# Kmatsuo57/cell-image-analysis

Measured on NVIDIA B200. Metric: cells scored/sec (crop+resize+CAE+SVM), higher is better.
Workload: dtype f16 tensor cores (CAE, PCA, SVM cross term: fp16 hi+lo operands, fp32 accumulate) / f64 norms and sums

## Files before the change

### cell-image-analysis_b200/csrc/cae_tc.cu

```cuda
#include "common.cuh"
#include "tc_ptx.cuh"

#include <cuda.h>
#include <cuda_fp16.h>

#include <cmath>

namespace {

constexpr int TCT = 256;
enum { EPI_POOL = 0, EPI_PLAIN = 2, EPI_FINAL = 3, EPI_PHASE = 4 };

using namespace tcptx;

#ifdef CIA_LANE0_ISSUE
#define ISSUE_WARP(cond) (lane == 0 && (cond))
#define ISSUE_BEGIN {
#define ISSUE_END }
#else
#define ISSUE_WARP(cond) (cond)
#define ISSUE_BEGIN if (elect_one()) {
#define ISSUE_END } __syncwarp();
#endif
#ifdef CIA_SPIN_WAIT
#define MBAR_WAIT mbar_wait
#else
#define MBAR_WAIT mbar_wait_sleep
#endif
#ifdef CIA_SLEEP_WAIT_ALL
#define mbar_wait mbar_wait_sleep
#endif
#ifdef CIA_UNIFORM_ISSUE_ALL
#define ISSUE1_WARP(cond) (cond)
#define ISSUE1_BEGIN if (elect_one()) {
#define ISSUE1_END } __syncwarp();
#else
#define ISSUE1_WARP(cond) (lane == 0 && (cond))
#define ISSUE1_BEGIN {
#define ISSUE1_END }
#endif

__device__ __forceinline__ float pooled_act(float folded_max, float inv_scale, float invd, float b, float s, float t) {
    const float m = __uint_as_float(__float_as_uint(folded_max) ^ (__float_as_uint(s) & 0x80000000u));
    return __fadd_rn(__fmul_rn(fmaxf(fmaf(m, inv_scale, fmaf(m, invd, b)), 0.f), s), t);
}

__device__ __forceinline__ void split_store8(const float (&o)[8], __half* hi_dst, __half* lo_dst, bool& range_ok) {
    __align__(16) __half hh[8];
    __align__(16) __half ll[8];
#pragma unroll
    for (int k = 0; k < 8; ++k) {
        hh[k] = __float2half_rn(o[k]);
        ll[k] = __float2half_rn(o[k] - __half2float(hh[k]));
        range_ok = range_ok && fabsf(o[k]) < 65520.f;
    }
    *reinterpret_cast<uint4*>(hi_dst) = *reinterpret_cast<const uint4*>(hh);
    if (lo_dst) *reinterpret_cast<uint4*>(lo_dst) = *reinterpret_cast<const uint4*>(ll);
}

template <int CIN, int COUT, int R, int EPI, int NPASS>
struct Cfg {
    static constexpr bool POOL = EPI == EPI_POOL;
    static constexpr int NCH = CIN / 8;
    static constexpr int FILL_ROWS = POOL ? R + 2 : 18;
    static constexpr int UNIT_COLS = (R >= 32 && CIN >= 64) ? 16 : R;
    static constexpr int COL_BLOCKS = R / UNIT_COLS;
    static constexpr int ROW_UNITS = POOL ? 9 : UNIT_COLS + 2;
    static constexpr int ROW_B = ROW_UNITS * 16;
    static constexpr int PLANE_B = FILL_ROWS * ROW_B;
    static constexpr int CHUNK_B = (POOL ? 2 : 1) * PLANE_B;
    static constexpr int REGION_B = NCH * CHUNK_B;
    static constexpr int SBO_A = POOL ? 2 * ROW_B : ROW_B;
    static constexpr int TILES = POOL ? 4 : (UNIT_COLS >= 8 ? UNIT_COLS / 8 : 1);
    static constexpr int UNITS_PER_CELL = POOL ? (R >= 32 ? 2 : 1) : (R >= 32 ? 2 : 1) * COL_BLOCKS;
    static constexpr int TBUF_COLS = TILES * COUT;
    static constexpr int TMEM_COLS = pow2_cols((NPASS == 1 ? 2 : 1) * TBUF_COLS);
    static constexpr int W_B = 9 * NCH * COUT * 16;
    static constexpr int PARTS = NPASS > 1 ? 2 : 1;
    static constexpr int SMEM_B = PARTS * (REGION_B + W_B);
    static constexpr bool DED_ISSUER = NPASS == 1 && !POOL && EPI != EPI_FINAL && SMEM_B > 100 * 1024;
    static constexpr int THREADS = TCT + (DED_ISSUER ? 32 : 0);
};

template <class C, int R, int NPASS, int NT, int BATCH, bool UPSIN = false>
__device__ __forceinline__ void stage_block(const __half* __restrict__ in_hi, const __half* __restrict__ in_lo,
                                            unsigned char* a0, unsigned char* a1, int cell, int sub, int tid) {
    constexpr int COLS = C::POOL ? 18 : C::ROW_UNITS;
    constexpr int N_UNITS16 = C::NCH * C::FILL_ROWS * COLS;
    constexpr int ITERS = (N_UNITS16 + NT - 1) / NT;
#pragma unroll 1
    for (int i0 = 0; i0 < ITERS; i0 += BATCH) {
        uint4 vh[BATCH], vl[BATCH];
        uint32_t dst[BATCH];
#pragma unroll
        for (int j = 0; j < BATCH; ++j) {
            const int idx = tid + (i0 + j) * NT;
            vh[j] = make_uint4(0, 0, 0, 0); vl[j] = make_uint4(0, 0, 0, 0);
            dst[j] = 0xFFFFFFFFu;
            if (i0 + j < ITERS && idx < N_UNITS16) {
                const int c = idx / (C::FILL_ROWS * COLS);
                const int rem = idx - c * (C::FILL_ROWS * COLS);
                const int ry = rem / COLS, rc = rem - ry * COLS;
                int y, x;
                if (C::POOL) {
                    y = ry - 1; x = 16 * sub - 1 + rc;
                    dst[j] = (uint32_t)(((c * 2 + (rc & 1)) * C::FILL_ROWS + ry) * 9 + (rc >> 1)) * 16u;
                } else {
                    y = 16 * (sub / C::COL_BLOCKS) + ry - 1;
                    x = C::UNIT_COLS * (sub % C::COL_BLOCKS) + rc - 1;
                    dst[j] = (uint32_t)((c * C::FILL_ROWS + ry) * C::ROW_UNITS + rc) * 16u;
                }
                if (y >= 0 && y < R && x >= 0 && x < R) {
                    constexpr int RS = UPSIN ? R / 2 : R;
                    const int ys = UPSIN ? (y >> 1) : y, xs = UPSIN ? (x >> 1) : x;
                    const size_t src = ((((size_t)cell * C::NCH + c) * RS + ys) * RS + xs);
                    vh[j] = __ldg(reinterpret_cast<const uint4*>(in_hi) + src);
                    if (NPASS > 1) vl[j] = __ldg(reinterpret_cast<const uint4*>(in_lo) + src);
                }
            }
        }
#pragma unroll
        for (int j = 0; j < BATCH; ++j) {
            if (dst[j] != 0xFFFFFFFFu) {
                *reinterpret_cast<uint4*>(a0 + dst[j]) = vh[j];
                if (NPASS > 1) *reinterpret_cast<uint4*>(a1 + dst[j]) = vl[j];
            }
        }
    }
}

template <int CIN, int COUT, int R, int EPI, int NPASS, bool UPSIN>
__global__ void __launch_bounds__(Cfg<CIN, COUT, R, EPI, NPASS>::THREADS, (Cfg<CIN, COUT, R, EPI, NPASS>::SMEM_B > 100 * 1024) ? 1 : 2)
conv_tc_kernel(const __half* __restrict__ in_hi, const __half* __restrict__ in_lo,
               const uint4* __restrict__ w_hi, const uint4* __restrict__ w_lo, float inv_scale,
               const float* __restrict__ bias, const float* __restrict__ bn_s,
               const float* __restrict__ bn_t, __half* __restrict__ out_hi, __half* __restrict__ out_lo,
               float* __restrict__ feat, const float* __restrict__ crops, float* __restrict__ mse,
               float* __restrict__ mae, int n_cells, const int32_t* __restrict__ n_dev, int cell0,
               int chunk_cells,
               int32_t* __restrict__ status) {
    bool range_ok = true;
    using C = Cfg<CIN, COUT, R, EPI, NPASS>;
    extern __shared__ __align__(1024) unsigned char smem[];
    __shared__ __align__(8) uint64_t bar[2];
    __shared__ uint32_t tmem_base_s;
    __shared__ float red_s[2][2][TCT / 32];

    const int tid = threadIdx.x, warp = tid >> 5, lane = tid & 31;
    unsigned char* a_part[2] = {smem, smem + C::REGION_B};
    unsigned char* w_part[2] = {smem + C::PARTS * C::REGION_B, smem + C::PARTS * C::REGION_B + C::W_B};

    int n = dev_count(n_cells, n_dev) - cell0;
    if (n > chunk_cells) n = chunk_cells;
    if (n <= 0) return;
    const int n_units = n * C::UNITS_PER_CELL;

    if (warp == 0) tmem_alloc(&tmem_base_s, C::TMEM_COLS);
    constexpr int NISS = C::DED_ISSUER ? 1 : C::TILES;
    if (tid == 32) { mbar_init(&bar[0], NISS); mbar_init(&bar[1], NISS); fence_barrier_init(); }
    for (int i = tid; i < C::W_B / 16; i += TCT) {
        reinterpret_cast<uint4*>(w_part[0])[i] = __ldg(w_hi + i);
        if (NPASS > 1) reinterpret_cast<uint4*>(w_part[1])[i] = __ldg(w_lo + i);
    }
    tc_fence_before();
    __syncthreads();
    tc_fence_after();
    const uint32_t tmem_base = tmem_base_s;
    constexpr uint32_t IDESC = make_idesc(128, COUT);

    constexpr int S_COLS = C::POOL ? 18 : C::ROW_UNITS;
    constexpr int S_N = C::NCH * C::FILL_ROWS * S_COLS;
    constexpr int S_IT = (S_N + TCT - 1) / TCT;
    constexpr bool PIPE = NPASS == 1;
    uint32_t s_dst[S_IT], s_crc[S_IT];
    uint4 s_val[S_IT];
    if (PIPE) {
#pragma unroll
        for (int j = 0; j < S_IT; ++j) {
            const int idx = tid + j * TCT;
            s_dst[j] = 0xFFFFFFFFu; s_crc[j] = 0;
            if (idx < S_N && tid < TCT) {
                const int c = idx / (C::FILL_ROWS * S_COLS);
                const int rem = idx - c * (C::FILL_ROWS * S_COLS);
                const int ry = rem / S_COLS, rc = rem - ry * S_COLS;
                s_crc[j] = (uint32_t)((c << 16) | (ry << 8) | rc);
                s_dst[j] = C::POOL ? (uint32_t)(((c * 2 + (rc & 1)) * C::FILL_ROWS + ry) * 9 + (rc >> 1)) * 16u
                                   : (uint32_t)((c * C::FILL_ROWS + ry) * C::ROW_UNITS + rc) * 16u;
            }
        }
    }
    auto prefetch = [&](int unit) {
        const int cell = cell0 + unit / C::UNITS_PER_CELL;
        const int sub = unit % C::UNITS_PER_CELL;
        const int y0 = C::POOL ? -1 : 16 * (sub / C::COL_BLOCKS) - 1;
        const int x0 = C::POOL ? 16 * sub - 1 : C::UNIT_COLS * (sub % C::COL_BLOCKS) - 1;
        constexpr int RS = UPSIN ? R / 2 : R;
        const uint4* base = reinterpret_cast<const uint4*>(in_hi) + (size_t)cell * C::NCH * RS * RS;
#pragma unroll
        for (int j = 0; j < S_IT; ++j) {
            const int c = (int)(s_crc[j] >> 16), y = y0 + (int)((s_crc[j] >> 8) & 255u), x = x0 + (int)(s_crc[j] & 255u);
            s_val[j] = make_uint4(0, 0, 0, 0);
            if (s_dst[j] != 0xFFFFFFFFu && y >= 0 && y < R && x >= 0 && x < R) {
                const int ys = UPSIN ? (y >> 1) : y, xs = UPSIN ? (x >> 1) : x;
                s_val[j] = __ldg(base + ((size_t)c * RS + ys) * RS + xs);
            }
        }
    };
    auto park = [&]() {
#pragma unroll
// ... 1302 lines not shown
}

namespace l7 {
constexpr int EPI_WARPS = 16;
constexpr int NT = (EPI_WARPS + 1) * 32;
constexpr int A_B = 1024 * 32 * 2;
constexpr int W_B = 4 * 32 * 16;
constexpr int PL_B = 16 * 1024 * 4;
constexpr int SMEM_B = 2 * A_B + W_B + PL_B;
constexpr int STAGE_COLS = 8 * 32;
}

__global__ void __launch_bounds__(l7::NT, 1)
final_tapsum_kernel(const __half* __restrict__ a6, const uint4* __restrict__ w_img, float inv_scale,
                    const float* __restrict__ bias, const float* __restrict__ crops,
                    float* __restrict__ mse, float* __restrict__ mae, int n_cells,
                    const int32_t* __restrict__ n_dev, int cell0, int chunk_cells) {
    using namespace l7;
    extern __shared__ __align__(1024) unsigned char smem[];
    __shared__ __align__(8) uint64_t a_full[2], d_full[2], d_empty[2];
    __shared__ uint32_t tmem_base_s;
    __shared__ float red_s[2][2][EPI_WARPS];
    unsigned char* const w_s = smem + 2 * A_B;
    float* const planes = reinterpret_cast<float*>(smem + 2 * A_B + W_B);

    const int tid = threadIdx.x, warp = tid >> 5, lane = tid & 31;
    int n = dev_count(n_cells, n_dev) - cell0;
    if (n > chunk_cells) n = chunk_cells;
    if (n <= 0) return;
    const int stride = (int)gridDim.x;

    if (warp == 0) tmem_alloc(&tmem_base_s, 2 * STAGE_COLS);
    if (tid == 32) {
        for (int i = 0; i < 2; ++i) { mbar_init(&a_full[i], 1); mbar_init(&d_full[i], 1); mbar_init(&d_empty[i], EPI_WARPS); }
        fence_barrier_init();
    }
    for (int i = tid; i < W_B / 16; i += NT) reinterpret_cast<uint4*>(w_s)[i] = __ldg(w_img + i);
    fence_async_smem();
    tc_fence_before();
    __syncthreads();
    tc_fence_after();
    const uint32_t tmem_base = tmem_base_s;

    if (warp == EPI_WARPS) {
        if (ISSUE1_WARP(true)) {
            constexpr uint32_t IDESC = make_idesc(128, 32);
            const uint64_t bd0 = make_smem_desc(smem_u32(w_s), 32 * 16, 128);
            const __half* src0 = a6 + (size_t)cell0 * (A_B / 2);
            ISSUE1_BEGIN
            for (int k = 0; k < 2; ++k) {
                const int unit = (int)blockIdx.x + k * stride;
                if (unit < n) {
                    mbar_expect_tx(&a_full[k], A_B);
                    bulk_load(smem_u32(smem) + k * A_B, src0 + (size_t)unit * (A_B / 2), A_B, &a_full[k]);
                }
            }
            ISSUE1_END
            uint32_t it = 0;
            for (int unit = blockIdx.x; unit < n; unit += stride, ++it) {
                const uint32_t st = it & 1, ph = (it >> 1) & 1;
                mbar_wait(&a_full[st], ph);
                mbar_wait(&d_empty[st], ph ^ 1);
                tc_fence_after();
                ISSUE1_BEGIN
                const uint64_t ad0 = make_smem_desc(smem_u32(smem) + st * A_B, 1024 * 16, 128);
#pragma unroll
                for (int t = 0; t < 8; ++t)
#pragma unroll
                    for (int ks = 0; ks < 2; ++ks)
                        umma_f16(tmem_base + st * STAGE_COLS + (uint32_t)(t * 32),
                                 ad0 + (uint64_t)((t * 128 * 16 + 2 * ks * 1024 * 16) >> 4),
                                 bd0 + (uint64_t)((2 * ks * 32 * 16) >> 4), IDESC, ks);
                umma_commit(&d_full[st]);
                ISSUE1_END
                mbar_wait(&d_full[st], ph);
                if (unit + 2 * stride < n) {
                    ISSUE1_BEGIN
                    mbar_expect_tx(&a_full[st], A_B);
                    bulk_load(smem_u32(smem) + st * A_B, src0 + (size_t)(unit + 2 * stride) * (A_B / 2), A_B, &a_full[st]);
                    ISSUE1_END
                }
            }
        }
    } else {
        const int q = warp & 3, g = warp >> 2;
        const float b = __ldg(bias);
        uint32_t it = 0;
        for (int unit = blockIdx.x; unit < n; unit += stride, ++it) {
            const uint32_t st = it & 1, ph = (it >> 1) & 1;
            const int cell = cell0 + unit;
            mbar_wait(&d_full[st], ph);
            tc_fence_after();
#pragma unroll
            for (int tt = 0; tt < 2; ++tt) {
                const int t = g + 4 * tt;
                const int p = 128 * t + 32 * q + lane;
                const uint32_t taddr = tmem_base + ((uint32_t)(32 * q) << 16) + st * STAGE_COLS + (uint32_t)(t * 32);
                uint32_t v[4][8];
#pragma unroll
                for (int k = 0; k < 4; ++k) TMEM_LD8(taddr + 8 * k, v[k]);
#pragma unroll
                for (int k = 0; k < 4; ++k) TMEM_WAIT8(v[k]);
#pragma unroll
                for (int c = 0; c < 16; ++c)
                    planes[c * 1024 + p] = __uint_as_float(v[c >> 3][c & 7]) + __uint_as_float(v[2 + (c >> 3)][c & 7]);
            }
            tc_fence_before();
            __syncwarp();
            if (lane == 0) mbar_arrive(&d_empty[st]);
            asm volatile("bar.sync 1, %0;" ::"n"(EPI_WARPS * 32) : "memory");
            float se = 0.f, ae = 0.f;
            const float* xr = crops + (size_t)cell * 4096;
#pragma unroll
            for (int tt = 0; tt < 2; ++tt) {
                const int p = 128 * (g + 4 * tt) + 32 * q + lane;
                const int Y = p >> 5, X = p & 31;
#pragma unroll
                for (int py = 0; py < 2; ++py) {
                    const float2 xv = __ldg(reinterpret_cast<const float2*>(xr + (2 * Y + py) * 64 + 2 * X));
#pragma unroll
                    for (int px = 0; px < 2; ++px) {
                        float sum = 0.f;
#pragma unroll
                        for (int ty = 0; ty < 2; ++ty)
#pragma unroll
                            for (int tx = 0; tx < 2; ++tx) {
                                const int yy = Y + py - 1 + ty, xx = X + px - 1 + tx;
                                if ((unsigned)yy < 32u && (unsigned)xx < 32u)
                                    sum += planes[(4 * (2 * py + px) + 2 * ty + tx) * 1024 + yy * 32 + xx];
                            }
                        const float a = fmaf(sum, inv_scale, b);
                        const float rec = __fdividef(1.f, 1.f + __expf(-a));
                        const float d = (px ? xv.y : xv.x) - rec;
                        se = fmaf(d, d, se);
                        ae += fabsf(d);
                    }
                }
            }
            se = warp_sum(se); ae = warp_sum(ae);
            if (lane == 0) { red_s[it & 1][0][warp] = se; red_s[it & 1][1][warp] = ae; }
            asm volatile("bar.sync 1, %0;" ::"n"(EPI_WARPS * 32) : "memory");
            if (tid == 0) {
                float s = 0.f, a = 0.f;
#pragma unroll
                for (int w = 0; w < EPI_WARPS; ++w) { s += red_s[it & 1][0][w]; a += red_s[it & 1][1][w]; }
                mse[cell] = s * (1.f / 4096.f);
                mae[cell] = a * (1.f / 4096.f);
            }
        }
    }
    tc_fence_before();
    __syncthreads();
    if (warp == 0) tmem_dealloc(tmem_base, 2 * l7::STAGE_COLS);
}

template <int CIN, int COUT, int R, int EPI, int NPASS, bool UPSIN = false>
int launch_tc(cia_ctx* h, const CaeWeights& w, int layer, const __half* in_hi, const __half* in_lo,
              __half* out_hi, __half* out_lo, float* feat, const float* crops, float* mse, float* mae,
              int n, const int32_t* n_dev, int cell0, int chunk, cudaStream_t s) {
    using C = Cfg<CIN, COUT, R, EPI, NPASS>;
    auto kern = conv_tc_kernel<CIN, COUT, R, EPI, NPASS, UPSIN>;
    if (first_use(h, (const void*)kern))
        CIA_CUDA(cudaFuncSetAttribute(kern, cudaFuncAttributeMaxDynamicSharedMemorySize, C::SMEM_B));
    int grid = chunk * C::UNITS_PER_CELL;
    const int cap = h->num_sms * (C::SMEM_B > 100 * 1024 ? 1 : 2);
    if (grid > cap) grid = cap;
    kern<<<grid, C::THREADS, C::SMEM_B, s>>>(in_hi, in_lo, (const uint4*)w.tc_w[layer][0], (const uint4*)w.tc_w[layer][1],
                                      w.tc_inv_scale[layer], w.bias[layer], w.bn_scale[layer], w.bn_shift[layer],
                                      out_hi, out_lo, feat, crops, mse, mae, n, n_dev, cell0, chunk, h->status_dev);
    CIA_LAUNCH_CHECK();
    return CIA_OK;
}

#ifdef CIA_ACC_TIMING
static void acc_timing_dump(const char* name, int cin, int cout, int r, int g, cudaStream_t s) {
    if (!getenv("CIA_ACC_DUMP")) return;
    unsigned long long d[16];
    cudaStreamSynchronize(s);
    cudaMemcpyFromSymbol(d, g_acc_dbg, sizeof(d));
    const double u = d[5] ? (double)d[5] : 1.0;
    fprintf(stderr, "%s<%d,%d,%d,G%d> cells %llu per-cell cycles: stage %.0f wait_full %.0f ld %.0f ld+add %.0f "
                    "final %.0f | mma: wait_ready %.0f wait_empty %.0f issue %.0f\n", name, cin, cout, r, g, d[5],
            d[0] / u, d[1] / u, d[2] / u, d[3] / u, d[4] / u, d[8] / u, d[9] / u, d[10] / u);
    memset(d, 0, sizeof(d));
    cudaMemcpyToSymbol(g_acc_dbg, d, sizeof(d));
}
#else
static inline void acc_timing_dump(const char*, int, int, int, int, cudaStream_t) {}
#endif

static float acc_debias(const cia_ctx* h, int layer) { return h->cae_debias[layer == 1 ? 1 : 2] * 5.9604645e-8f; }

template <int CIN, int COUT, int R, int G = 1>
int launch_tc_acc(cia_ctx* h, const CaeWeights& w, int layer, const __half* in_hi, const __half* in_lo,
                  __half* out_hi, __half* out_lo, float* feat, int n, const int32_t* n_dev, int cell0,
                  int chunk, cudaStream_t s) {
    using C = AccCfg<CIN, COUT, R>;
    auto kern = conv_tc_acc_kernel<CIN, COUT, R, G>;
    if (first_use(h, (const void*)kern))
        CIA_CUDA(cudaFuncSetAttribute(kern, cudaFuncAttributeMaxDynamicSharedMemorySize, C::SMEM_B));
    int grid = chunk;
    if (grid > h->num_sms) grid = h->num_sms;
    kern<<<grid, ACC_THREADS, C::SMEM_B, s>>>(in_hi, in_lo, (const uint4*)w.tc_w[layer][0],
                                              (const uint4*)w.tc_w[layer][1], w.tc_inv_scale[layer],
                                              w.tc_inv_scale[layer] * acc_debias(h, layer), w.bias[layer],
                                              w.bn_scale[layer], w.bn_shift[layer], out_hi, out_lo, feat, n, n_dev,
                                              cell0, chunk, h->status_dev);
    CIA_LAUNCH_CHECK();
    acc_timing_dump("acc", CIN, COUT, R, G, s);
    return CIA_OK;
}

typedef CUresult (*TensorMapEncodeFn)(CUtensorMap*, CUtensorMapDataType, cuuint32_t, void*, const cuuint64_t*,
                                      const cuuint64_t*, const cuuint32_t*, const cuuint32_t*, CUtensorMapInterleave,
                                      CUtensorMapSwizzle, CUtensorMapL2promotion, CUtensorMapFloatOOBfill);

static int encode_act_map(cia_ctx* h, CUtensorMap* tm, const __half* base, int nch, int r, int cells, int box_x,
                          int box_y) {
    static TensorMapEncodeFn encode = [] {
        void* fn = nullptr;
        cudaDriverEntryPointQueryResult q;
        if (cudaGetDriverEntryPoint("cuTensorMapEncodeTiled", &fn, cudaEnableDefault, &q) != cudaSuccess) fn = nullptr;
        return (TensorMapEncodeFn)fn;
    }();
    if (!encode) { h->err = "cuTensorMapEncodeTiled is not available from this driver"; return CIA_E_UNSUPPORTED; }
    const cuuint64_t dims[5] = {8, (cuuint64_t)r, (cuuint64_t)r, (cuuint64_t)nch, (cuuint64_t)cells};
    const cuuint64_t strides[4] = {16, (cuuint64_t)16 * r, (cuuint64_t)16 * r * r, (cuuint64_t)16 * r * r * nch};
    const cuuint32_t box[5] = {8, (cuuint32_t)box_x, (cuuint32_t)box_y, (cuuint32_t)nch, 1};
    const cuuint32_t estr[5] = {1, 2, 1, 1, 1};
    const CUresult rc = encode(tm, CU_TENSOR_MAP_DATA_TYPE_FLOAT16, 5, (void*)base, dims, strides, box, estr,
                               CU_TENSOR_MAP_INTERLEAVE_NONE, CU_TENSOR_MAP_SWIZZLE_NONE,
                               CU_TENSOR_MAP_L2_PROMOTION_L2_128B, CU_TENSOR_MAP_FLOAT_OOB_FILL_NONE);
    if (rc != CUDA_SUCCESS) { h->err = "cuTensorMapEncodeTiled failed"; return CIA_E_CUDA; }
    return CIA_OK;
}

template <int CIN, int COUT, int R, int G>
int launch_tc_acc2(cia_ctx* h, const CaeWeights& w, int layer, const __half* in_hi, const __half* in_lo,
                   int buf_cells, __half* out_hi, __half* out_lo, float* feat, int n, const int32_t* n_dev,
                   int cell0, int chunk, cudaStream_t s) {
    using C = Acc2Cfg<CIN, COUT, R>;
    static_assert(C::SMEM_B + 1280 <= 227 * 1024, "double-buffered blocks do not fit in shared memory");
    auto kern = conv_tc_acc2_kernel<CIN, COUT, R, G>;
    if (first_use(h, (const void*)kern))
        CIA_CUDA(cudaFuncSetAttribute(kern, cudaFuncAttributeMaxDynamicSharedMemorySize, C::SMEM_B));
    CUtensorMap tm_hi, tm_lo;
    int rc;
    if ((rc = encode_act_map(h, &tm_hi, in_hi, C::NCH, C::R, buf_cells, C::BOX_X, C::FILL_ROWS))) return rc;
    if ((rc = encode_act_map(h, &tm_lo, in_lo, C::NCH, C::R, buf_cells, C::BOX_X, C::FILL_ROWS))) return rc;
    int grid = chunk;
    if (grid > h->num_sms) grid = h->num_sms;
    kern<<<grid, ACC_THREADS, C::SMEM_B, s>>>(tm_hi, tm_lo, (const uint4*)w.tc_w[layer][0],
                                              (const uint4*)w.tc_w[layer][1], w.tc_inv_scale[layer],
                                              w.tc_inv_scale[layer] * acc_debias(h, layer), w.bias[layer],
                                              w.bn_scale[layer], w.bn_shift[layer], out_hi, out_lo, feat, n, n_dev,
                                              cell0, chunk, h->status_dev);
    CIA_LAUNCH_CHECK();
    acc_timing_dump("acc2", CIN, COUT, R, G, s);
    return CIA_OK;
}

template <int G, int VAR = 0>
int launch_l2_stack(cia_ctx* h, const CaeWeights& w, const __half* in_hi, const __half* in_lo, int buf_cells,
                    __half* out_hi, __half* out_lo, float* feat, int n, const int32_t* n_dev, int cell0, int chunk,
                    cudaStream_t s) {
    using C = Acc2Cfg<32, 64, 32>;
    auto kern = conv_tc_l2_stack_kernel<G, VAR>;
    if (first_use(h, (const void*)kern))
        CIA_CUDA(cudaFuncSetAttribute(kern, cudaFuncAttributeMaxDynamicSharedMemorySize, C::SMEM_B));
    CUtensorMap tm_hi, tm_lo;
    int rc;
    if ((rc = encode_act_map(h, &tm_hi, in_hi, C::NCH, C::R, buf_cells, C::BOX_X, C::FILL_ROWS))) return rc;
    if ((rc = encode_act_map(h, &tm_lo, in_lo, C::NCH, C::R, buf_cells, C::BOX_X, C::FILL_ROWS))) return rc;
    int grid = chunk;
    if (grid > h->num_sms) grid = h->num_sms;
    kern<<<grid, ACC_THREADS, C::SMEM_B, s>>>(tm_hi, tm_lo, (const uint4*)w.tc_w[1][0], (const uint4*)w.tc_w[1][1],
                                              w.tc_inv_scale[1], w.tc_inv_scale[1] * acc_debias(h, 1), w.bias[1],
                                              w.bn_scale[1], w.bn_shift[1], out_hi, out_lo, feat, n, n_dev, cell0, chunk, h->status_dev);
    CIA_LAUNCH_CHECK();
    return CIA_OK;
}

static void pack_image(const std::vector<float>& w , int taps, int cin, int N,
                       int n_real, int sw, std::vector<__half>& hi, std::vector<__half>& lo,
                       const float* colsign = nullptr) {
    const int nch = cin / 8;
    hi.assign((size_t)taps * nch * N * 8, __float2half_rn(0.f));
    lo = hi;
    const float sc = std::ldexp(1.f, sw);
    for (int tap = 0; tap < taps; ++tap)
        for (int c = 0; c < cin; ++c)
            for (int nn = 0; nn < n_real; ++nn) {
                const float v = w[((size_t)tap * cin + c) * n_real + nn] * sc * (colsign ? colsign[nn] : 1.f);
                const __half hv = __float2half_rn(v);
                const size_t idx = (((size_t)tap * nch + c / 8) * N + nn) * 8 + (c % 8);
                hi[idx] = hv;
                lo[idx] = __float2half_rn(v - __half2float(hv));
            }
}

static int scale_exp(const std::vector<float>& w) {
    float m = 0.f;
    for (float v : w) m = std::fmax(m, std::fabs(v));
    if (!(m > 0.f)) return 0;
    int e;
    std::frexp(m, &e);
// ... 61 lines not shown
                                    kt[(size_t)c * 16 + 4 * (2 * py + px) + 2 * ty + tx] += k[((size_t)(dy * 3 + dx) * cin + c)];
                            }
                std::vector<__half> img((size_t)(cin / 8) * 32 * 8, __float2half_rn(0.f));
                const float sc = std::ldexp(1.f, sw);
                for (int c = 0; c < cin; ++c)
                    for (int col = 0; col < 16; ++col) {
                        const float v = kt[(size_t)c * 16 + col] * sc;
                        const __half hv = __float2half_rn(v);
                        img[((size_t)(c / 8) * 32 + col) * 8 + (c % 8)] = hv;
                        img[((size_t)(c / 8) * 32 + 16 + col) * 8 + (c % 8)] = __float2half_rn(v - __half2float(hv));
                    }
                cudaFree(w.tc_w7); w.tc_w7 = nullptr;
                CIA_CUDA(cudaMalloc(&w.tc_w7, img.size() * sizeof(__half)));
                CIA_CUDA(cudaMemcpy(w.tc_w7, img.data(), img.size() * sizeof(__half), cudaMemcpyHostToDevice));
            }
        } else if (L == 5) {
            const int N = 4 * cout;
            std::vector<float> kp((size_t)9 * cin * N, 0.f);
            for (int py = 0; py < 2; ++py)
                for (int px = 0; px < 2; ++px)
                    for (int dy = 0; dy < 3; ++dy)
                        for (int dx = 0; dx < 3; ++dx) {
                            const int oy = (int)std::floor((py + dy - 1) / 2.0), ox = (int)std::floor((px + dx - 1) / 2.0);
                            const int tl = (oy + 1) * 3 + (ox + 1);
                            for (int c = 0; c < cin; ++c)
                                for (int co = 0; co < cout; ++co)
                                    kp[((size_t)tl * cin + c) * N + (py * 2 + px) * cout + co] +=
                                        k[((size_t)(dy * 3 + dx) * cin + c) * cout + co];
                        }
            sw = scale_exp(kp);
            pack_image(kp, 9, cin, N, N, sw, hi, lo);
        } else {
            sw = scale_exp(k);
            pack_image(k, 9, cin, cout, cout, sw, hi, lo, L < 3 ? colsign.data() : nullptr);
        }
        w.tc_inv_scale[L] = std::ldexp(1.f, -sw);
        for (int j = 0; j < 2; ++j) {
            cudaFree(w.tc_w[L][j]); w.tc_w[L][j] = nullptr;
            const std::vector<__half>& src = j == 0 ? hi : lo;
            CIA_CUDA(cudaMalloc(&w.tc_w[L][j], src.size() * sizeof(__half)));
            CIA_CUDA(cudaMemcpy(w.tc_w[L][j], src.data(), src.size() * sizeof(__half), cudaMemcpyHostToDevice));
        }
    }
    w.tc_ready = true;
    return CIA_OK;
}

int k_cae_forward_tc(cia_ctx* h, const float* crops, int n, const int32_t* n_dev, float* mse,
                     float* mae, float* features, int mode, cudaStream_t s) {
    if (n <= 0) return CIA_OK;
    const CaeWeights& ae = h->cae[0];
    if (!ae.loaded || ae.n_conv != 7 || !ae.tc_ready) { h->err = "cia_cae_forward: autoencoder not loaded"; return CIA_E_STATE; }
    const bool sep = h->cae[1].loaded;
    const bool tc_feat = mode == 1 && !sep;
    const bool l3_exact = mode == 3 && !sep;
    const int CH_MAX = h->cae_pass_cells;
    const int CH = n < CH_MAX ? (n + 147) / 148 * 148 : CH_MAX;
    const size_t a1 = 4 * 32 * 32 * 8, a2 = 8 * 16 * 16 * 8, a3 = 4 * 8 * 8 * 8, a4u = 4 * 8 * 8 * 8,
                 a5u = 8 * 16 * 16 * 8, a6 = 4 * 32 * 32 * 8;
    const size_t per_cell = 2 * a1 + 2 * a2 + a3 + a4u + a5u + a6;
    int rc = ws_reserve(h, h->ws_misc, (size_t)CH * per_cell * sizeof(__half));
    if (rc) return rc;
    float* A2f = nullptr;
    if (l3_exact) {
        if ((rc = ws_reserve(h, h->ws_act, (size_t)CH * 16 * 16 * 64 * sizeof(float)))) return rc;
        A2f = (float*)h->ws_act.p;
    }
    __half* A1h = (__half*)h->ws_misc.p;
    __half* A1l = A1h + CH * a1;
    __half* A2h = A1l + CH * a1;
    __half* A2l = A2h + CH * a2;
    __half* A3h = A2l + CH * a2;
    __half* A4u = A3h + CH * a3;
    __half* A5u = A4u + CH * a4u;
    __half* A6 = A5u + CH * a5u;
    CIA_CUDA(cudaMemsetAsync(mse, 0, (size_t)n * sizeof(float), s));
    CIA_CUDA(cudaMemsetAsync(mae, 0, (size_t)n * sizeof(float), s));
    const bool side_encoder = features && !tc_feat && !l3_exact;
    if (side_encoder) {
        CIA_CUDA(cudaEventRecord(h->ev_fork, s));
        CIA_CUDA(cudaStreamWaitEvent(h->side, h->ev_fork, 0));
        rc = k_encoder_fp32(h, sep ? h->cae[1] : h->cae[0], crops, n, n_dev, features, h->side);
        if (rc) return rc;
        CIA_CUDA(cudaEventRecord(h->ev_join, h->side));
    }
    for (int c0 = 0; c0 < n; c0 += CH) {
        const int chunk = (n - c0) < CH ? (n - c0) : CH;
        __half* a1h = A1h - (size_t)c0 * a1; __half* a1l = A1l - (size_t)c0 * a1;
        __half* a2h = A2h - (size_t)c0 * a2; __half* a2l = A2l - (size_t)c0 * a2;
        __half* a3h = A3h - (size_t)c0 * a3; __half* a4 = A4u - (size_t)c0 * a4u;
        __half* a5 = A5u - (size_t)c0 * a5u; __half* a6p = A6 - (size_t)c0 * a6;
        float* feat = tc_feat ? features : nullptr;
        int grid1 = chunk * 4;
        if (grid1 > h->num_sms * 8) grid1 = h->num_sms * 8;
        const int pass = c0 / CH;
        if (h->layer_ev && pass < CIA_LAYER_PASSES) h->layer_passes = pass + 1;
#define CIA_LMARK(i) do { if (h->layer_ev && pass < CIA_LAYER_PASSES) CIA_CUDA(cudaEventRecord(h->layer_ev[pass * CIA_LAYER_MARKS + (i)], s)); } while (0)
        CIA_LMARK(0);
        if (tc_feat || l3_exact) {
            static const int l1_tc = [] { const char* e = getenv("CIA_L1_KERNEL"); return e ? atoi(e) : 1; }();
            const float l1_debias = h->cae_debias[0] * 5.9604645e-8f;
            if (l1_tc) {
                if (first_use(h, (const void*)conv1_tc_split_kernel))
                    CIA_CUDA(cudaFuncSetAttribute(conv1_tc_split_kernel, cudaFuncAttributeMaxDynamicSharedMemorySize, l1tc::SMEM_B));
                int gridt = chunk * 8;
                if (gridt > h->num_sms * 2) gridt = h->num_sms * 2;
                conv1_tc_split_kernel<<<gridt, l1tc::NT, l1tc::SMEM_B, s>>>(crops, (const uint4*)ae.tc_w[0][0], ae.tc_inv_scale[0],
                                                                            l1_debias, ae.bias[0], ae.bn_scale[0], ae.bn_shift[0],
                                                                            a1h, a1l, n, n_dev, c0, chunk, h->status_dev);
            } else {
                conv1_fp32_planar_kernel<<<grid1, 256, 0, s>>>(crops, ae.kernel[0], ae.bias[0], ae.bn_scale[0],
                                                               ae.bn_shift[0], a1h, a1l, n, n_dev, c0, chunk, h->status_dev);
            }
            CIA_LAUNCH_CHECK();
            CIA_LMARK(1);
            float* a2f = l3_exact ? A2f - (size_t)c0 * (16 * 16 * 64) : nullptr;
            static const int l2_g = [] { const char* e = getenv("CIA_L2_TAPS_PER_FLUSH"); return e ? atoi(e) : 3; }();
            static const int l2_stack = [] { const char* e = getenv("CIA_L2_STACK"); return e ? atoi(e) : 0; }();
            if (l2_stack == 2 && l2_g == 3) rc = launch_l2_stack<3, 1>(h, ae, A1h, A1l, CH, a2h, a2l, a2f, n, n_dev, c0, chunk, s);
            else if (l2_stack == 3 && l2_g == 3) rc = launch_l2_stack<3, 2>(h, ae, A1h, A1l, CH, a2h, a2l, a2f, n, n_dev, c0, chunk, s);
            else if (l2_stack && l2_g == 3) rc = launch_l2_stack<3>(h, ae, A1h, A1l, CH, a2h, a2l, a2f, n, n_dev, c0, chunk, s);
            else if (l2_g == 0) rc = launch_tc_acc<32, 64, 32, 1>(h, ae, 1, a1h, a1l, a2h, a2l, a2f, n, n_dev, c0, chunk, s);
            else if (l2_g == 1) rc = launch_tc_acc2<32, 64, 32, 1>(h, ae, 1, A1h, A1l, CH, a2h, a2l, a2f, n, n_dev, c0, chunk, s);
            else if (l2_g == 9) rc = launch_tc_acc2<32, 64, 32, 9>(h, ae, 1, A1h, A1l, CH, a2h, a2l, a2f, n, n_dev, c0, chunk, s);
            else if (l2_g == 2) rc = launch_tc_acc2<32, 64, 32, 2>(h, ae, 1, A1h, A1l, CH, a2h, a2l, a2f, n, n_dev, c0, chunk, s);
            else rc = launch_tc_acc2<32, 64, 32, 3>(h, ae, 1, A1h, A1l, CH, a2h, a2l, a2f, n, n_dev, c0, chunk, s);
            if (rc) return rc;
            CIA_LMARK(2);
            if (l3_exact) {
                if ((rc = launch_tc<64, 32, 16, EPI_POOL, 1>(h, ae, 2, a2h, nullptr, a3h, nullptr, nullptr, nullptr, nullptr, nullptr, n, n_dev, c0, chunk, s))) return rc;
                if (features && (rc = k_conv3_fp32(h, ae, a2f, n, n_dev, features, c0, chunk, s))) return rc;
            } else {
                static const int l3_tma = [] { const char* e = getenv("CIA_L3_KERNEL"); return e ? atoi(e) : 0; }();
                static const int l3_g = [] { const char* e = getenv("CIA_L3_TAPS_PER_FLUSH"); return e ? atoi(e) : 1; }();
                if (l3_tma) rc = launch_tc_acc2<64, 32, 16, 1>(h, ae, 2, A2h, A2l, CH, a3h, nullptr, feat, n, n_dev, c0, chunk, s);
                else if (l3_g == 3) rc = launch_tc_acc<64, 32, 16, 3>(h, ae, 2, a2h, a2l, a3h, nullptr, feat, n, n_dev, c0, chunk, s);
                else rc = launch_tc_acc<64, 32, 16, 1>(h, ae, 2, a2h, a2l, a3h, nullptr, feat, n, n_dev, c0, chunk, s);
                if (rc) return rc;
            }
        } else {
            conv1_fp32_planar_kernel<<<grid1, 256, 0, s>>>(crops, ae.kernel[0], ae.bias[0], ae.bn_scale[0],
                                                           ae.bn_shift[0], a1h, nullptr, n, n_dev, c0, chunk, h->status_dev);
            CIA_LAUNCH_CHECK();
            CIA_LMARK(1);
            if ((rc = launch_tc<32, 64, 32, EPI_POOL, 1>(h, ae, 1, a1h, nullptr, a2h, nullptr, nullptr, nullptr, nullptr, nullptr, n, n_dev, c0, chunk, s))) return rc;
            CIA_LMARK(2);
            if ((rc = launch_tc<64, 32, 16, EPI_POOL, 1>(h, ae, 2, a2h, nullptr, a3h, nullptr, nullptr, nullptr, nullptr, nullptr, n, n_dev, c0, chunk, s))) return rc;
        }
        CIA_LMARK(3);
        if ((rc = launch_tc<32, 32, 8, EPI_PLAIN, 1>(h, ae, 3, a3h, nullptr, a4, nullptr, nullptr, nullptr, nullptr, nullptr, n, n_dev, c0, chunk, s))) return rc;
        CIA_LMARK(4);
        if ((rc = launch_tc<32, 64, 16, EPI_PLAIN, 1, true>(h, ae, 4, a4, nullptr, a5, nullptr, nullptr, nullptr, nullptr, nullptr, n, n_dev, c0, chunk, s))) return rc;
        CIA_LMARK(5);
        if ((rc = launch_tc<64, 128, 16, EPI_PHASE, 1>(h, ae, 5, a5, nullptr, a6p, nullptr, nullptr, nullptr, nullptr, nullptr, n, n_dev, c0, chunk, s))) return rc;
        CIA_LMARK(6);
        static const int l7_tapsum = [] { const char* e = getenv("CIA_L7_KERNEL"); return e ? atoi(e) : 1; }();
        if (l7_tapsum) {
            if (first_use(h, (const void*)final_tapsum_kernel))
                CIA_CUDA(cudaFuncSetAttribute(final_tapsum_kernel, cudaFuncAttributeMaxDynamicSharedMemorySize, l7::SMEM_B));
            int g7 = chunk < h->num_sms ? chunk : h->num_sms;
            final_tapsum_kernel<<<g7, l7::NT, l7::SMEM_B, s>>>(a6p, (const uint4*)ae.tc_w7, ae.tc_inv_scale[6], ae.bias[6],
                                                              crops, mse, mae, n, n_dev, c0, chunk);
            CIA_LAUNCH_CHECK();
        } else if ((rc = launch_tc<32, 16, 32, EPI_FINAL, 1>(h, ae, 6, a6p, nullptr, nullptr, nullptr, nullptr, crops, mse, mae, n, n_dev, c0, chunk, s))) return rc;
        CIA_LMARK(7);
#undef CIA_LMARK
    }
    if (side_encoder) CIA_CUDA(cudaStreamWaitEvent(s, h->ev_join, 0));
    return CIA_OK;
}
```

### cell-image-analysis_b200/csrc/tc_ptx.cuh

```cuda
#pragma once
#include <cuda_runtime.h>
#include <stdint.h>

namespace tcptx {

__device__ __forceinline__ uint32_t smem_u32(const void* p) { return (uint32_t)__cvta_generic_to_shared(p); }

__device__ __forceinline__ void mbar_init(uint64_t* bar, uint32_t count) {
    asm volatile("mbarrier.init.shared::cta.b64 [%0], %1;" ::"r"(smem_u32(bar)), "r"(count) : "memory");
}
__device__ __forceinline__ void mbar_wait(uint64_t* bar, uint32_t parity) {
    const uint32_t a = smem_u32(bar);
    uint32_t done;
    do {
        asm volatile(
            "{\n\t.reg .pred p;\n\t"
            "mbarrier.try_wait.parity.shared::cta.b64 p, [%1], %2;\n\t"
            "selp.u32 %0, 1, 0, p;\n\t}"
            : "=r"(done) : "r"(a), "r"(parity) : "memory");
    } while (!done);
}
__device__ __forceinline__ void mbar_wait_sleep(uint64_t* bar, uint32_t parity) {
    const uint32_t a = smem_u32(bar);
    asm volatile(
        "{\n\t.reg .pred p;\n\t"
        "WAIT_%=:\n\t"
        "mbarrier.try_wait.parity.shared::cta.b64 p, [%0], %1, %2;\n\t"
        "@p bra DONE_%=;\n\t"
        "bra WAIT_%=;\n\t"
        "DONE_%=:\n\t}"
        ::"r"(a), "r"(parity), "r"(0x989680u) : "memory");
}
__device__ __forceinline__ bool elect_one() {
    uint32_t pred;
    asm volatile("{\n\t.reg .pred p;\n\telect.sync _|p, 0xffffffff;\n\tselp.u32 %0, 1, 0, p;\n\t}" : "=r"(pred));
    return pred != 0;
}
__device__ __forceinline__ void fence_barrier_init() { asm volatile("fence.mbarrier_init.release.cluster;" ::: "memory"); }
__device__ __forceinline__ void fence_async_smem() { asm volatile("fence.proxy.async.shared::cta;" ::: "memory"); }
__device__ __forceinline__ void tc_fence_before() { asm volatile("tcgen05.fence::before_thread_sync;" ::: "memory"); }
__device__ __forceinline__ void tc_fence_after() { asm volatile("tcgen05.fence::after_thread_sync;" ::: "memory"); }

__device__ __forceinline__ void tmem_alloc(uint32_t* dst_smem, uint32_t ncols) {
    asm volatile("tcgen05.alloc.cta_group::1.sync.aligned.shared::cta.b32 [%0], %1;" ::"r"(smem_u32(dst_smem)), "r"(ncols) : "memory");
    asm volatile("tcgen05.relinquish_alloc_permit.cta_group::1.sync.aligned;" ::: "memory");
}
__device__ __forceinline__ void tmem_dealloc(uint32_t taddr, uint32_t ncols) {
    asm volatile("tcgen05.dealloc.cta_group::1.sync.aligned.b32 %0, %1;" ::"r"(taddr), "r"(ncols) : "memory");
}
__device__ __forceinline__ void umma_f16(uint32_t d_tmem, uint64_t adesc, uint64_t bdesc, uint32_t idesc,
                                         uint32_t accumulate) {
    asm volatile(
        "{\n\t.reg .pred p;\n\tsetp.ne.b32 p, %4, 0;\n\t"
        "tcgen05.mma.cta_group::1.kind::f16 [%0], %1, %2, %3, p;\n\t}"
        ::"r"(d_tmem), "l"(adesc), "l"(bdesc), "r"(idesc), "r"(accumulate) : "memory");
}
__device__ __forceinline__ void umma_commit(uint64_t* bar) {
    asm volatile("tcgen05.commit.cta_group::1.mbarrier::arrive::one.shared::cluster.b64 [%0];" ::"r"(smem_u32(bar)) : "memory");
}
#define TMEM_LD8(taddr, v)                                                                          \
    asm volatile("tcgen05.ld.sync.aligned.32x32b.x8.b32 {%0,%1,%2,%3,%4,%5,%6,%7}, [%8];"            \
                 : "=r"(v[0]), "=r"(v[1]), "=r"(v[2]), "=r"(v[3]), "=r"(v[4]), "=r"(v[5]), "=r"(v[6]), \
                   "=r"(v[7]) : "r"(taddr))
#define TMEM_WAIT8(v)                                                                               \
    asm volatile("tcgen05.wait::ld.sync.aligned;"                                                   \
                 : "+r"(v[0]), "+r"(v[1]), "+r"(v[2]), "+r"(v[3]), "+r"(v[4]), "+r"(v[5]), "+r"(v[6]), \
                   "+r"(v[7]) :: "memory")

#define TMEM_LD16(taddr, v)                                                                               \
    asm volatile("tcgen05.ld.sync.aligned.32x32b.x16.b32 "                                                \
                 "{%0,%1,%2,%3,%4,%5,%6,%7,%8,%9,%10,%11,%12,%13,%14,%15}, [%16];"                         \
                 : "=r"(v[0]), "=r"(v[1]), "=r"(v[2]), "=r"(v[3]), "=r"(v[4]), "=r"(v[5]), "=r"(v[6]),     \
                   "=r"(v[7]), "=r"(v[8]), "=r"(v[9]), "=r"(v[10]), "=r"(v[11]), "=r"(v[12]), "=r"(v[13]), \
                   "=r"(v[14]), "=r"(v[15]) : "r"(taddr))
#define TMEM_WAIT16(v)                                                                                    \
    asm volatile("tcgen05.wait::ld.sync.aligned;"                                                         \
                 : "+r"(v[0]), "+r"(v[1]), "+r"(v[2]), "+r"(v[3]), "+r"(v[4]), "+r"(v[5]), "+r"(v[6]),     \
                   "+r"(v[7]), "+r"(v[8]), "+r"(v[9]), "+r"(v[10]), "+r"(v[11]), "+r"(v[12]), "+r"(v[13]), \
                   "+r"(v[14]), "+r"(v[15]) :: "memory")

__device__ __forceinline__ uint64_t make_smem_desc(uint32_t saddr, uint32_t lbo_bytes, uint32_t sbo_bytes) {
    uint64_t d = 0;
    d |= (uint64_t)((saddr >> 4) & 0x3FFFu);
    d |= (uint64_t)((lbo_bytes >> 4) & 0x3FFFu) << 16;
    d |= (uint64_t)((sbo_bytes >> 4) & 0x3FFFu) << 32;
    d |= (uint64_t)1 << 46;
    return d;
}
__host__ __device__ constexpr uint32_t make_idesc(int M, int N) {
    return (1u << 4) | ((uint32_t)(N >> 3) << 17) | ((uint32_t)(M >> 4) << 24);
}
__host__ __device__ constexpr int pow2_cols(int c) { return c <= 32 ? 32 : c <= 64 ? 64 : c <= 128 ? 128 : c <= 256 ? 256 : 512; }

__device__ __forceinline__ void mbar_arrive(uint64_t* bar) {
    asm volatile("mbarrier.arrive.shared::cta.b64 _, [%0];" ::"r"(smem_u32(bar)) : "memory");
}

__device__ __forceinline__ void mbar_expect_tx(uint64_t* bar, uint32_t bytes) {
    asm volatile("mbarrier.arrive.expect_tx.shared::cta.b64 _, [%0], %1;" ::"r"(smem_u32(bar)), "r"(bytes) : "memory");
}
__device__ __forceinline__ void bulk_load(uint32_t dst, const void* src, uint32_t bytes, uint64_t* bar) {
    asm volatile("cp.async.bulk.shared::cluster.global.mbarrier::complete_tx::bytes [%0], [%1], %2, [%3];"
                 ::"r"(dst), "l"(src), "r"(bytes), "r"(smem_u32(bar)) : "memory");
}


__device__ __forceinline__ unsigned long long pack2(float lo, float hi) {
    unsigned long long r;
    asm("mov.b64 %0, {%1,%2};" : "=l"(r) : "f"(lo), "f"(hi));
    return r;
}
__device__ __forceinline__ void unpack2(unsigned long long v, float& lo, float& hi) {
    asm("mov.b64 {%0,%1}, %2;" : "=f"(lo), "=f"(hi) : "l"(v));
}
__device__ __forceinline__ unsigned long long fma2(unsigned long long a, unsigned long long b, unsigned long long c) {
    unsigned long long d;
    asm("fma.rn.f32x2 %0, %1, %2, %3;" : "=l"(d) : "l"(a), "l"(b), "l"(c));
    return d;
}
__device__ __forceinline__ void fadd2(float& a0, float& a1, uint32_t b0, uint32_t b1) {
    asm("{\n\t.reg .b64 ra, rb;\n\tmov.b64 ra, {%0,%1};\n\tmov.b64 rb, {%2,%3};\n\t"
        "add.rn.f32x2 ra, ra, rb;\n\tmov.b64 {%0,%1}, ra;\n\t}"
        : "+f"(a0), "+f"(a1) : "r"(b0), "r"(b1));
}


}
```

Measured before the change: 3.175 million.

## Fuse decoder conv6 and final tapsum layer into one persistent tcgen05 kernel

Adds a persistent kernel that runs the layer-6 conv on tensor cores and, in the same CTA, feeds the fp16 layer-6 output straight from shared memory into the layer-7 tapsum MMA, the sigmoid and the per-cell MSE/MAE reduction. The L7 MMAs are interleaved into the L6 issue loop via a non-blocking mbarrier test, and TMEM is double-buffered. This removes one kernel launch and the round trip of the layer-6 activations through global memory as the L7 input, while overlapping L6 compute with the L7 epilogue. It still writes a6p to global (the copy is now unused), takes one CTA per SM with large shared memory, and adds complex synchronisation that could mis-order work.

```diff
diff --git a/cell-image-analysis_b200/csrc/cae_tc.cu b/cell-image-analysis_b200/csrc/cae_tc.cu
--- a/cell-image-analysis_b200/csrc/cae_tc.cu
+++ b/cell-image-analysis_b200/csrc/cae_tc.cu
@@ -45,7 +45,8 @@
     return __fadd_rn(__fmul_rn(fmaxf(fmaf(m, inv_scale, fmaf(m, invd, b)), 0.f), s), t);
 }
 
-__device__ __forceinline__ void split_store8(const float (&o)[8], __half* hi_dst, __half* lo_dst, bool& range_ok) {
+__device__ __forceinline__ void split_store8(const float (&o)[8], __half* hi_dst, __half* lo_dst, bool& range_ok,
+                                             unsigned char* hi_copy = nullptr ) {
     __align__(16) __half hh[8];
     __align__(16) __half ll[8];
 #pragma unroll
@@ -55,6 +56,7 @@
         range_ok = range_ok && fabsf(o[k]) < 65520.f;
     }
     *reinterpret_cast<uint4*>(hi_dst) = *reinterpret_cast<const uint4*>(hh);
+    if (hi_copy) *reinterpret_cast<uint4*>(hi_copy) = *reinterpret_cast<const uint4*>(hh);
     if (lo_dst) *reinterpret_cast<uint4*>(lo_dst) = *reinterpret_cast<const uint4*>(ll);
 }
 
@@ -1663,6 +1665,283 @@
     tc_fence_before();
     __syncthreads();
     if (warp == 0) tmem_dealloc(tmem_base, 2 * l7::STAGE_COLS);
+}
+
+namespace l67 {
+using C = Cfg<64, 128, 16, EPI_PHASE, 1>;
+constexpr int NT = C::THREADS;
+constexpr int T_B = 4 * 4 * 128 * 16;
+constexpr int T_OFF = C::REGION_B + C::W_B;
+constexpr int SEAM_OFF = T_OFF + T_B + l7::W_B;
+constexpr int SMEM_B = SEAM_OFF + 16 * 32 * 4;
+static_assert(C::DED_ISSUER && C::UNITS_PER_CELL == 1 && C::TILES == 2 && C::TMEM_COLS == 512, "L6 geometry");
+static_assert(SMEM_B <= 232448, "shared memory per block");
+}
+
+__global__ void __launch_bounds__(l67::NT, 1)
+conv6_final_kernel(const __half* __restrict__ in_hi, const uint4* __restrict__ w6, float inv_scale6,
+                   const float* __restrict__ bias6, const float* __restrict__ bn_s, const float* __restrict__ bn_t,
+                   __half* __restrict__ a6, const uint4* __restrict__ w7, float inv_scale7,
+                   const float* __restrict__ bias7, const float* __restrict__ crops, float* __restrict__ mse,
+                   float* __restrict__ mae, int n_cells, const int32_t* __restrict__ n_dev, int cell0,
+                   int chunk_cells, int32_t* __restrict__ status) {
+    using namespace l67;
+    bool range_ok = true;
+    extern __shared__ __align__(1024) unsigned char smem[];
+    __shared__ __align__(8) uint64_t bar[2], l7_ready, l7_done;
+    __shared__ uint32_t tmem_base_s;
+    __shared__ float red_s[2][2][TCT / 32];
+    unsigned char* const a_s = smem;
+    unsigned char* const w6_s = smem + C::REGION_B;
+    unsigned char* const t_s = smem + T_OFF;
+    float* const planes = reinterpret_cast<float*>(t_s);
+    unsigned char* const w7_s = t_s + T_B;
+    float* const seam = reinterpret_cast<float*>(smem + SEAM_OFF);
+
+    const int tid = threadIdx.x, warp = tid >> 5, lane = tid & 31;
+    int n = dev_count(n_cells, n_dev) - cell0;
+    if (n > chunk_cells) n = chunk_cells;
+    if (n <= 0) return;
+    const int stride = (int)gridDim.x;
+
+    if (warp == 0) tmem_alloc(&tmem_base_s, C::TMEM_COLS);
+    if (tid == 32) {
+        mbar_init(&bar[0], 1); mbar_init(&bar[1], 1);
+        mbar_init(&l7_ready, TCT / 32); mbar_init(&l7_done, 1);
+        fence_barrier_init();
+    }
+    for (int i = tid; i < C::W_B / 16; i += NT) reinterpret_cast<uint4*>(w6_s)[i] = __ldg(w6 + i);
+    for (int i = tid; i < l7::W_B / 16; i += NT) reinterpret_cast<uint4*>(w7_s)[i] = __ldg(w7 + i);
+    fence_async_smem();
+    tc_fence_before();
+    __syncthreads();
+    tc_fence_after();
+    const uint32_t tmem_base = tmem_base_s;
+
+    constexpr int S_N = C::NCH * C::FILL_ROWS * C::ROW_UNITS;
+    constexpr int S_IT = (S_N + TCT - 1) / TCT;
+    uint32_t s_crc[S_IT];
+    uint4 s_val[S_IT];
+#pragma unroll
+    for (int j = 0; j < S_IT; ++j) {
+        const int idx = tid + j * TCT;
+        s_crc[j] = 0xFFFFFFFFu;
+        if (idx < S_N && tid < TCT) {
+            const int c = idx / (C::FILL_ROWS * C::ROW_UNITS);
+            const int rem = idx - c * (C::FILL_ROWS * C::ROW_UNITS);
+            const int ry = rem / C::ROW_UNITS, rc = rem - ry * C::ROW_UNITS;
+            s_crc[j] = (uint32_t)((c << 16) | (ry << 8) | rc);
+        }
+    }
+    auto prefetch = [&](int unit) {
+        const uint4* base = reinterpret_cast<const uint4*>(in_hi) + (size_t)(cell0 + unit) * C::NCH * 16 * 16;
+#pragma unroll
+        for (int j = 0; j < S_IT; ++j) {
+            const int c = (int)(s_crc[j] >> 16), y = (int)((s_crc[j] >> 8) & 255u) - 1, x = (int)(s_crc[j] & 255u) - 1;
+            s_val[j] = make_uint4(0, 0, 0, 0);
+            if (s_crc[j] != 0xFFFFFFFFu && y >= 0 && y < 16 && x >= 0 && x < 16)
+                s_val[j] = __ldg(base + ((size_t)c * 16 + y) * 16 + x);
+        }
+    };
+    auto park = [&]() {
+#pragma unroll
+        for (int j = 0; j < S_IT; ++j)
+            if (s_crc[j] != 0xFFFFFFFFu) reinterpret_cast<uint4*>(a_s)[tid + j * TCT] = s_val[j];
+    };
+    auto issue_l7 = [&](uint32_t tb, int t) {
+        constexpr uint32_t IDESC = make_idesc(128, 32);
+        const uint64_t ad0 = make_smem_desc(smem_u32(t_s), 128 * 16, 128);
+        const uint64_t bd0 = make_smem_desc(smem_u32(w7_s), 32 * 16, 128);
+#pragma unroll
+        for (int ph = 0; ph < 4; ++ph)
+#pragma unroll
+            for (int ks = 0; ks < 2; ++ks)
+                umma_f16(tmem_base + tb * C::TBUF_COLS + (uint32_t)(t * 128 + ph * 32),
+                         ad0 + (uint64_t)((ph * 4 * 128 * 16 + 2 * ks * 128 * 16) >> 4),
+                         bd0 + (uint64_t)((2 * ks * 32 * 16) >> 4), IDESC, ks);
+        umma_commit(&l7_done);
+    };
+    auto issue_l6 = [&](uint32_t tb, int l7_next) -> int {
+        constexpr uint32_t IDESC = make_idesc(128, 128);
+        const uint64_t ad0 = make_smem_desc(smem_u32(a_s), C::CHUNK_B, C::SBO_A);
+        const uint64_t bd0 = make_smem_desc(smem_u32(w6_s), 128 * 16, 128);
+#pragma unroll
+        for (int tap = 0; tap < 9; ++tap) {
+            const int dy = tap / 3, dx = tap % 3;
+#pragma unroll
+            for (int s = 0; s < 4; ++s)
+#pragma unroll
+                for (int t = 0; t < 2; ++t)
+                    umma_f16(tmem_base + tb * C::TBUF_COLS + (uint32_t)(t * 128),
+                             ad0 + (uint64_t)((t * 8 * 16 + dx * 16 + dy * C::ROW_B + 2 * s * C::CHUNK_B) >> 4),
+                             bd0 + (uint64_t)(((tap * C::NCH + 2 * s) * 128 * 16) >> 4), IDESC,
+                             (tap == 0 && s == 0) ? 0u : 1u);
+            if (l7_next < 2 && mbar_test(&l7_ready, (uint32_t)l7_next)) {
+                tc_fence_after();
+                issue_l7(tb ^ 1, l7_next++);
+            }
+        }
+        umma_commit(&bar[tb]);
+        return l7_next;
+    };
+
+    const int q = warp & 3, hs = (warp >> 2) & 1, r = 32 * q + lane;
+    const float b7 = __ldg(bias7);
+
+    if ((int)blockIdx.x < n) {
+        prefetch(blockIdx.x);
+        park();
+        fence_async_smem();
+        __syncthreads();
+        if (warp == TCT / 32 && lane == 0) { tc_fence_after(); issue_l6(0, 2); }
+        if ((int)blockIdx.x + stride < n) prefetch(blockIdx.x + stride);
+    }
+
+    uint32_t it = 0;
+    for (int unit = blockIdx.x; unit < n; unit += stride, ++it) {
+        const int cell = cell0 + unit;
+        const uint32_t tbuf = it & 1;
+        const bool more = unit + stride < n;
+        mbar_wait(&bar[tbuf], (it >> 1) & 1);
+        tc_fence_after();
+        if (more) {
+            park();
+            fence_async_smem();
+            tc_fence_before();
+            __syncthreads();
+        }
+        if (warp == TCT / 32) {
+            if (lane == 0) {
+                tc_fence_after();
+                int l7_next = more ? issue_l6(tbuf ^ 1, 0) : 0;
+                for (; l7_next < 2; ++l7_next) {
+                    mbar_wait(&l7_ready, (uint32_t)l7_next);
+                    tc_fence_after();
+                    issue_l7(tbuf, l7_next);
+                }
+            }
+            __syncwarp();
+            continue;
+        }
+        if (more && unit + 2 * stride < n) prefetch(unit + 2 * stride);
+
+        const uint32_t lane_addr = tmem_base + ((uint32_t)(32 * q) << 16) + tbuf * C::TBUF_COLS;
+        const float* xr = crops + (size_t)cell * 4096;
+        float se = 0.f, ae = 0.f;
+#pragma unroll 1
+        for (int t = 0; t < 2; ++t) {
+            float2 xv[2][2];
+#pragma unroll
+            for (int k = 0; k < 2; ++k) {
+                const int p = tid + TCT * k, Y = p >> 4, X = 16 * t + (p & 15);
+#pragma unroll
+                for (int py = 0; py < 2; ++py)
+                    xv[k][py] = __ldg(reinterpret_cast<const float2*>(xr + (2 * Y + py) * 64 + 2 * X));
+            }
+            float xs[2] = {0.f, 0.f};
+            if (t == 1 && tid < 32) {
+                xs[0] = __ldg(xr + (2 * tid) * 64 + 31);
+                xs[1] = __ldg(xr + (2 * tid + 1) * 64 + 31);
+            }
+            const int y = r >> 3, x = 8 * t + (r & 7);
+#pragma unroll
+            for (int j = 0; j < 2; ++j) {
+                const int cs = hs + 2 * j;
+                uint32_t v[4][8];
+#pragma unroll
+                for (int ph = 0; ph < 4; ++ph) TMEM_LD8(lane_addr + (uint32_t)(t * 128 + ph * 32 + cs * 8), v[ph]);
+                float b8[8], s8[8], t8[8];
+#pragma unroll
+                for (int k = 0; k < 8; ++k) {
+                    b8[k] = __ldg(bias6 + cs * 8 + k); s8[k] = __ldg(bn_s + cs * 8 + k); t8[k] = __ldg(bn_t + cs * 8 + k);
+                }
+#pragma unroll
+                for (int ph = 0; ph < 4; ++ph) TMEM_WAIT8(v[ph]);
+#pragma unroll
+                for (int ph = 0; ph < 4; ++ph) {
+                    float o[8];
+#pragma unroll
+                    for (int k = 0; k < 8; ++k) {
+                        const float a = fmaxf(fmaf(__uint_as_float(v[ph][k]), inv_scale6, b8[k]), 0.f);
+                        o[k] = __fadd_rn(__fmul_rn(a, s8[k]), t8[k]);
+                    }
+                    const size_t off = ((((size_t)cell * 4 + cs) * 32 + 2 * y + (ph >> 1)) * 32 + 2 * x + (ph & 1)) * 8;
+                    split_store8(o, a6 + off, nullptr, range_ok, t_s + ((ph * 4 + cs) * 128 + r) * 16);
+                }
+            }
+            fence_async_smem();
+            tc_fence_before();
+            __syncwarp();
+            if (lane == 0) mbar_arrive(&l7_ready);
+            mbar_wait(&l7_done, (uint32_t)t);
+            tc_fence_after();
+#pragma unroll
+            for (int j = 0; j < 2; ++j) {
+                const int ph = 2 * hs + j;
+                uint32_t v[4][8];
+#pragma unroll
+                for (int k = 0; k < 4; ++k) TMEM_LD8(lane_addr + (uint32_t)(t * 128 + ph * 32 + 8 * k), v[k]);
+#pragma unroll
+                for (int k = 0; k < 4; ++k) TMEM_WAIT8(v[k]);
+#pragma unroll
+                for (int c = 0; c < 16; ++c) {
+                    const float p = __uint_as_float(v[c >> 3][c & 7]) + __uint_as_float(v[2 + (c >> 3)][c & 7]);
+                    planes[(c * 4 + ph) * 128 + r] = p;
+                    if (t == 0 && (ph & 1) && (r & 7) == 7) seam[c * 32 + 2 * (r >> 3) + (ph >> 1)] = p;
+                }
+            }
+            tc_fence_before();
+            asm volatile("bar.sync 1, %0;" ::"n"(TCT) : "memory");
+            auto P = [&](int yy, int xx, int col) -> float {
+                if (xx < 16 * t) return seam[col * 32 + yy];
+                const int xl = xx - 16 * t;
+                return planes[(col * 4 + (yy & 1) * 2 + (xl & 1)) * 128 + 8 * (yy >> 1) + (xl >> 1)];
+            };
+            auto output = [&](int Y, int X, int py, int px, float xval) {
+                float sum = 0.f;
+#pragma unroll
+                for (int ty = 0; ty < 2; ++ty)
+#pragma unroll
+                    for (int tx = 0; tx < 2; ++tx) {
+                        const int yy = Y + py - 1 + ty, xx = X + px - 1 + tx;
+                        if ((unsigned)yy < 32u && (unsigned)xx < 32u) sum += P(yy, xx, 4 * (2 * py + px) + 2 * ty + tx);
+                    }
+                const float a = fmaf(sum, inv_scale7, b7);
+                const float rec = __fdividef(1.f, 1.f + __expf(-a));
+                const float d = xval - rec;
+                se = fmaf(d, d, se);
+                ae += fabsf(d);
+            };
+#pragma unroll
+            for (int k = 0; k < 2; ++k) {
+                const int p = tid + TCT * k, Y = p >> 4, X = 16 * t + (p & 15);
+#pragma unroll
+                for (int py = 0; py < 2; ++py)
+#pragma unroll
+                    for (int px = 0; px < 2; ++px)
+                        if (t == 1 || X != 15 || px == 0) output(Y, X, py, px, px ? xv[k][py].y : xv[k][py].x);
+            }
+            if (t == 1 && tid < 32) {
+                output(tid, 15, 0, 1, xs[0]);
+                output(tid, 15, 1, 1, xs[1]);
+            }
+            if (t == 0) asm volatile("bar.sync 1, %0;" ::"n"(TCT) : "memory");
+        }
+        se = warp_sum(se); ae = warp_sum(ae);
+        if (lane == 0) { red_s[it & 1][0][warp] = se; red_s[it & 1][1][warp] = ae; }
+        asm volatile("bar.sync 1, %0;" ::"n"(TCT) : "memory");
+        if (tid == 0) {
+            float s = 0.f, a = 0.f;
+#pragma unroll
+            for (int w = 0; w < TCT / 32; ++w) { s += red_s[it & 1][0][w]; a += red_s[it & 1][1][w]; }
+            mse[cell] = s * (1.f / 4096.f);
+            mae[cell] = a * (1.f / 4096.f);
+        }
+    }
+    tc_fence_before();
+    __syncthreads();
+    if (warp == 0) tmem_dealloc(tmem_base, C::TMEM_COLS);
+    if (!range_ok) raise_status(status, CIA_E_UNSUPPORTED);
 }
 
 template <int CIN, int COUT, int R, int EPI, int NPASS, bool UPSIN = false>
@@ -2030,17 +2309,30 @@
         CIA_LMARK(4);
         if ((rc = launch_tc<32, 64, 16, EPI_PLAIN, 1, true>(h, ae, 4, a4, nullptr, a5, nullptr, nullptr, nullptr, nullptr, nullptr, n, n_dev, c0, chunk, s))) return rc;
         CIA_LMARK(5);
-        if ((rc = launch_tc<64, 128, 16, EPI_PHASE, 1>(h, ae, 5, a5, nullptr, a6p, nullptr, nullptr, nullptr, nullptr, nullptr, n, n_dev, c0, chunk, s))) return rc;
-        CIA_LMARK(6);
         static const int l7_tapsum = [] { const char* e = getenv("CIA_L7_KERNEL"); return e ? atoi(e) : 1; }();
-        if (l7_tapsum) {
-            if (first_use(h, (const void*)final_tapsum_kernel))
-                CIA_CUDA(cudaFuncSetAttribute(final_tapsum_kernel, cudaFuncAttributeMaxDynamicSharedMemorySize, l7::SMEM_B));
-            int g7 = chunk < h->num_sms ? chunk : h->num_sms;
-            final_tapsum_kernel<<<g7, l7::NT, l7::SMEM_B, s>>>(a6p, (const uint4*)ae.tc_w7, ae.tc_inv_scale[6], ae.bias[6],
-                                                              crops, mse, mae, n, n_dev, c0, chunk);
+        static const int dec_fused = [] { const char* e = getenv("CIA_DECODER_FUSED"); return e ? atoi(e) : 1; }();
+        if (l7_tapsum && dec_fused) {
+            if (first_use(h, (const void*)conv6_final_kernel))
+                CIA_CUDA(cudaFuncSetAttribute(conv6_final_kernel, cudaFuncAttributeMaxDynamicSharedMemorySize, l67::SMEM_B));
+            const int g = chunk < h->num_sms ? chunk : h->num_sms;
+            conv6_final_kernel<<<g, l67::NT, l67::SMEM_B, s>>>(a5, (const uint4*)ae.tc_w[5][0], ae.tc_inv_scale[5], ae.bias[5],
+                                                               ae.bn_scale[5], ae.bn_shift[5], a6p, (const uint4*)ae.tc_w7,
+                                                               ae.tc_inv_scale[6], ae.bias[6], crops, mse, mae, n, n_dev, c0,
+                                                               chunk, h->status_dev);
             CIA_LAUNCH_CHECK();
-        } else if ((rc = launch_tc<32, 16, 32, EPI_FINAL, 1>(h, ae, 6, a6p, nullptr, nullptr, nullptr, nullptr, crops, mse, mae, n, n_dev, c0, chunk, s))) return rc;
+            CIA_LMARK(6);
+        } else {
+            if ((rc = launch_tc<64, 128, 16, EPI_PHASE, 1>(h, ae, 5, a5, nullptr, a6p, nullptr, nullptr, nullptr, nullptr, nullptr, n, n_dev, c0, chunk, s))) return rc;
+            CIA_LMARK(6);
+            if (l7_tapsum) {
+                if (first_use(h, (const void*)final_tapsum_kernel))
+                    CIA_CUDA(cudaFuncSetAttribute(final_tapsum_kernel, cudaFuncAttributeMaxDynamicSharedMemorySize, l7::SMEM_B));
+                int g7 = chunk < h->num_sms ? chunk : h->num_sms;
+                final_tapsum_kernel<<<g7, l7::NT, l7::SMEM_B, s>>>(a6p, (const uint4*)ae.tc_w7, ae.tc_inv_scale[6], ae.bias[6],
+                                                                  crops, mse, mae, n, n_dev, c0, chunk);
+                CIA_LAUNCH_CHECK();
+            } else if ((rc = launch_tc<32, 16, 32, EPI_FINAL, 1>(h, ae, 6, a6p, nullptr, nullptr, nullptr, nullptr, crops, mse, mae, n, n_dev, c0, chunk, s))) return rc;
+        }
         CIA_LMARK(7);
 #undef CIA_LMARK
     }
diff --git a/cell-image-analysis_b200/csrc/tc_ptx.cuh b/cell-image-analysis_b200/csrc/tc_ptx.cuh
--- a/cell-image-analysis_b200/csrc/tc_ptx.cuh
+++ b/cell-image-analysis_b200/csrc/tc_ptx.cuh
@@ -19,6 +19,15 @@
             "selp.u32 %0, 1, 0, p;\n\t}"
             : "=r"(done) : "r"(a), "r"(parity) : "memory");
     } while (!done);
+}
+__device__ __forceinline__ bool mbar_test(uint64_t* bar, uint32_t parity) {
+    uint32_t done;
+    asm volatile(
+        "{\n\t.reg .pred p;\n\t"
+        "mbarrier.test_wait.parity.shared::cta.b64 p, [%1], %2;\n\t"
+        "selp.u32 %0, 1, 0, p;\n\t}"
+        : "=r"(done) : "r"(smem_u32(bar)), "r"(parity) : "memory");
+    return done != 0;
 }
 __device__ __forceinline__ void mbar_wait_sleep(uint64_t* bar, uint32_t parity) {
     const uint32_t a = smem_u32(bar);
```

Measured after the change: 3.005 million, median of 6. 5.4% lower.
